# Anttwo/SuGaR

Measured on AMD Instinct MI355X. Metric: train_step_images_per_sec, higher is better.
Workload: dtype f32; 1 GPU; metric: 1000000 Gaussians @ 1920x1080, SH degree 3, 3DGS train step (raster fwd -> 0.8 L1 + 0.2 DSSIM -> bwd -> Adam, 59 floats/Gaussian), 8 orbit cameras cycled; parallelism=view-sharded dp1, single process, no collective

## Files before the change

### include/sugar_raster.h

```cpp
#ifndef SUGAR_RASTER_H_INCLUDED
#define SUGAR_RASTER_H_INCLUDED

#include <stddef.h>
#include <stdint.h>

#ifdef __cplusplus
extern "C" {
#endif

#define SGR_ABI_VERSION 4

#define SGR_E_INVALID (-1)
#define SGR_E_HIP (-2)
#define SGR_E_ALLOC (-3)

typedef char* (*sgr_alloc_fn)(void* user, size_t bytes);

int sgr_abi_version(void);
const char* sgr_last_error(void);

int64_t sgr_forward(sgr_alloc_fn geom_alloc, void* geom_user,
                    sgr_alloc_fn binning_alloc, void* binning_user,
                    sgr_alloc_fn img_alloc, void* img_user,
                    int P, int D, int M,
// ... 89 lines not shown
    float* campos_row;
    int flags;
} sgr_backward_opts;
#define SGR_BWD_EXACT_ALPHA 2
#define SGR_BWD_TILE_ORDER_READY 1
#define SGR_BWD_DENSE 8
#define SGR_BWD_ACC_CLEAN 4
#define SGR_BWD_ROWS_BY_REACH 16
#define SGR_BWD_ROWS_UNKNOWN 32
int sgr_backward_ex(int phase, int P, int D, int M, int64_t R,
                    const float* background, int width, int height,
                    const float* means3D, const float* shs, const float* colors_precomp,
                    const float* scales, float scale_modifier, const float* rotations,
                    const float* cov3D_precomp, const float* viewmatrix, const float* projmatrix,
                    const float* cam_pos, float tan_fovx, float tan_fovy, const int* radii,
                    char* geom_buffer, char* binning_buffer, char* img_buffer,
                    const float* dL_dpix,
                    float* dL_dmean2D, float* dL_dconic, float* dL_dopacity, float* dL_dcolor,
                    float* dL_dmean3D, float* dL_dcov3D, float* dL_dsh, float* dL_dscale, float* dL_drot,
                    int debug, void* stream, const sgr_backward_opts* opts);

int sgr_sh_grad_from_views(int P, int n_views, int D, int M, const float* means3D, const float* campos_all,
                           const float* dcolor_all, int64_t view_stride, float* dL_dsh, void* stream);

int sgr_sh_adam_from_views(int P, int n_views, int D, int M, const float* means3D, const float* campos_all,
                           const float* dcolor_all, int64_t view_stride, float* sh_params, float* exp_avg, float* exp_avg_sq,
                           float lr_dc,
                           float lr_rest, float beta1, float beta2, float eps, int step, float grad_scale, void* stream);

int sgr_sh_adam_from_views_ex(int P, int n_views, int D, int M, const float* means3D, const float* campos_all,
                              const float* dcolor_all, int64_t view_stride, float* sh_params, float* exp_avg, float* exp_avg_sq,
                              float lr_dc, float lr_rest, float beta1, float beta2, float eps, int step, float grad_scale,
                              float* dmean_extra, void* stream);

int sgr_sh_adam_zero_grad(int P, int M, float* sh_params, float* exp_avg, float* exp_avg_sq, const uint8_t* reach, float lr_dc,
                          float lr_rest, float beta1, float beta2, float eps, int step, float grad_scale,
                          const uint32_t* guard_header, uint32_t guard_capacity, void* stream);
int sgr_sh_adam_zero_grad_persistent(int P, int M, float* sh_params, float* exp_avg, float* exp_avg_sq, const uint8_t* reach, float lr_dc,
                                     float lr_rest, float beta1, float beta2, float eps, int step, float grad_scale,
                                     const uint32_t* guard_header, uint32_t guard_capacity, int n_adam, void* stream);
int sgr_sh_adam_from_views_masked(int P, int n_views, int D, int M, const float* means3D, const float* campos_all,
                                  const float* dcolor_all, int64_t view_stride, float* sh_params, float* exp_avg, float* exp_avg_sq,
                                  float lr_dc, float lr_rest, float beta1, float beta2, float eps, int step, float grad_scale,
                                  uint8_t* reach, const uint32_t* guard_header, uint32_t guard_capacity, void* stream);
void sgr_set_adam_overlap(int on);
int sgr_get_adam_overlap(void);
size_t sgr_geom_reach_offset_bytes(int P);
void sgr_set_rows_by_reach(int on);
int sgr_get_rows_by_reach(void);
size_t sgr_geom_rowdirty_offset_bytes(int P);

int sgr_mark_visible(int P, const float* means3D, const float* viewmatrix, const float* projmatrix,
                     uint8_t* present, void* stream);

size_t sgr_geom_bytes(int P);
size_t sgr_img_bytes(int width, int height);
size_t sgr_binning_bytes(int64_t R, int width, int height);

size_t sgr_geom_rec_offset(int P);
size_t sgr_geom_acc_offset_bytes(int P);
size_t sgr_img_final_T_offset(int width, int height);
size_t sgr_img_n_contrib_offset(int width, int height);
size_t sgr_img_tile_start_offset(int width, int height);
size_t sgr_img_tile_maxc_offset(int width, int height);
size_t sgr_img_tile_walked_offset(int width, int height);
size_t sgr_img_header_offset(int width, int height);
size_t sgr_binning_point_list_offset(int64_t R);

#define SGR_N_STAGES 15
void sgr_profile_enable(int stage_mask);
int sgr_profile_read(double* ms_sum, int64_t* count, int n_stages);


int sgr_dist2(int P, const float* points, float* meanDists, void* stream);
int sgr_knn(int N, const float* query, int M, const float* ref, int K, float* dists, int64_t* idx, void* stream);
size_t sgr_knn_grid_scratch_bytes(int M);
int sgr_knn_grid(int N, const float* query, int M, const float* ref, int K, float* dists, int64_t* idx, char* scratch,
                 void* stream);
int sgr_dist2_grid(int P, const float* points, float* meanDists, char* scratch, void* stream);

size_t sgr_l1_ssim_scratch_bytes(int channels, int width, int height);
int sgr_l1_ssim_forward(int channels, int width, int height, const float* img, const float* gt, float lambda,
                        char* scratch, float* loss_out, void* stream);
int sgr_l1_ssim_backward(int channels, int width, int height, const float* img, const float* gt, float lambda,
                         const char* scratch, const float* grad_loss, float* grad_img, void* stream);
int sgr_l1_ssim_backward_ex(int channels, int width, int height, const float* img, const float* gt, float lambda,
                            const char* scratch, const float* grad_loss, float* grad_img, float* loss_out, void* stream);

int sgr_adam_step(long long n, float* params, const float* grads, float* exp_avg, float* exp_avg_sq, int n_seg,
                  const long long* seg_begin, const long long* seg_end, const float* seg_lr_a, const float* seg_lr_b,
                  const int* seg_period, const int* seg_split, float beta1, float beta2, float eps, int step,
                  float grad_scale, void* stream);
int sgr_adam_step_multi(int n_tensors, const long long* n, float* const* params, const float* const* grads, float* const* exp_avg,
                        float* const* exp_avg_sq, const float* lr, const float* beta1, const float* beta2, const float* eps,
                        const int* step, void* stream);
int sgr_adam_step_ex(long long n, float* params, const float* grads, float* exp_avg, float* exp_avg_sq, int n_seg,
                     const long long* seg_begin, const long long* seg_end, const float* seg_lr_a, const float* seg_lr_b,
                     const int* seg_period, const int* seg_split, float beta1, float beta2, float eps, int step,
                     float grad_scale, const float* extra, long long extra_n, void* stream);

typedef struct sgr_train_config {
    int P, D, M, width, height;
    float* flat; float* flat_grad; float* exp_avg; float* exp_avg_sq;
    long long off_xyz, off_opacity, off_scaling, off_rotation, off_features, n_small;
    float lr_xyz, lr_opacity, lr_scaling, lr_rotation, lr_features_dc, lr_features_rest;
    float beta1, beta2, eps, lambda_dssim;
// ... 281 lines not shown
```

### sugar_amd/_lib.py

```python
from __future__ import annotations

import ctypes as C
import os

_HERE = os.path.dirname(os.path.abspath(__file__))
LIB_PATH = os.environ.get("SGR_LIB_PATH") or os.path.join(_HERE, "libsugar_raster.so")

ALLOC_FN = C.CFUNCTYPE(C.c_void_p, C.c_void_p, C.c_size_t)

_vp, _i, _f, _i64, _sz = C.c_void_p, C.c_int, C.c_float, C.c_int64, C.c_size_t
SIGNATURES = {
    "sgr_abi_version": (_i, []),
    "sgr_last_error": (C.c_char_p, []),
    "sgr_set_deep_min": (None, [_i]),
    "sgr_get_deep_min": (_i, []),
    "sgr_set_exact_alpha": (None, [_i]),
    "sgr_get_exact_alpha": (_i, []),
    "sgr_forward": (_i64, [ALLOC_FN, _vp, ALLOC_FN, _vp, ALLOC_FN, _vp, _i, _i, _i, _vp, _i, _i, _vp, _vp, _vp, _vp,
                           _vp, _f, _vp, _vp, _vp, _vp, _vp, _f, _f, _i, _vp, _vp, _i, _vp]),
    "sgr_forward_ex": (_i64, [ALLOC_FN, _vp, ALLOC_FN, _vp, ALLOC_FN, _vp, _i, _i, _i, _vp, _i, _i, _vp, _vp, _vp, _vp,
                              _vp, _f, _vp, _vp, _vp, _vp, _vp, _f, _f, _i, _vp, _vp, _i, _vp, _vp]),
    "sgr_backward": (_i, [_i, _i, _i, _i64, _vp, _i, _i, _vp, _vp, _vp, _vp, _f, _vp, _vp, _vp, _vp, _vp, _f, _f, _vp,
                          _vp, _vp, _vp, _vp, _vp, _vp, _vp, _vp, _vp, _vp, _vp, _vp, _vp, _i, _vp]),
    "sgr_backward_phase": (_i, [_i, _i, _i, _i, _i64, _vp, _i, _i, _vp, _vp, _vp, _vp, _f, _vp, _vp, _vp, _vp, _vp, _f, _f, _vp,
                                _vp, _vp, _vp, _vp, _vp, _vp, _vp, _vp, _vp, _vp, _vp, _vp, _vp, _i, _vp]),
    "sgr_backward_ex": (_i, [_i, _i, _i, _i, _i64, _vp, _i, _i, _vp, _vp, _vp, _vp, _f, _vp, _vp, _vp, _vp, _vp, _f, _f, _vp,
                             _vp, _vp, _vp, _vp, _vp, _vp, _vp, _vp, _vp, _vp, _vp, _vp, _vp, _i, _vp, _vp]),
    "sgr_mark_visible": (_i, [_i, _vp, _vp, _vp, _vp, _vp]),
    "sgr_trainer_create": (_vp, [_vp]),
    "sgr_trainer_destroy": (None, [_vp]),
    "sgr_trainer_set_binning": (_i, [_vp, _vp, _sz, _i64]),
    "sgr_trainer_step": (_i, [_vp, _vp, _i, _vp, _vp]),
    "sgr_trainer_forward_valid": (_i, [_vp, _vp]),
    "sgr_trainer_last_error": (C.c_char_p, []),
    "sgr_trainer_acc_dirty": (_i, [_vp]),
    "sgr_rccl_unique_id": (_i, [_vp]),
    "sgr_trainer_comm_init": (_i, [_vp, _vp, _i, _i, _vp, _sz]),
    "sgr_trainer_comm_destroy": (_i, [_vp]),
    "sgr_trainer_comm_abort": (_i, [_vp]),
    "sgr_trainer_step_exchange": (_i, [_vp, _vp, _i, _vp]),
    "sgr_trainer_set_exchange_chunks": (_i, [_vp, _i]),
    "sgr_trainer_last_exchange_wait_ms": (C.c_double, [_vp]),
    "sgr_bin2_bytes": (_sz, [_i, _i, _i]),
    "sgr_sh_grad_from_views": (_i, [_i, _i, _i, _i, _vp, _vp, _vp, _i64, _vp, _vp]),
    "sgr_sh_adam_from_views": (_i, [_i, _i, _i, _i, _vp, _vp, _vp, _i64, _vp, _vp, _vp, _f, _f, _f, _f, _f, _i, _f, _vp]),
    "sgr_sh_adam_from_views_ex": (_i, [_i, _i, _i, _i, _vp, _vp, _vp, _i64, _vp, _vp, _vp, _f, _f, _f, _f, _f, _i, _f, _vp, _vp]),
    "sgr_sh_adam_zero_grad": (_i, [_i, _i, _vp, _vp, _vp, _vp, _f, _f, _f, _f, _f, _i, _f, _vp, C.c_uint32, _vp]),
    "sgr_sh_adam_zero_grad_persistent": (_i, [_i, _i, _vp, _vp, _vp, _vp, _f, _f, _f, _f, _f, _i, _f, _vp, C.c_uint32, _i, _vp]),
    "sgr_sh_adam_from_views_masked": (_i, [_i, _i, _i, _i, _vp, _vp, _vp, _i64, _vp, _vp, _vp, _f, _f, _f, _f, _f, _i, _f, _vp, _vp,
                                           C.c_uint32, _vp]),
    "sgr_set_adam_overlap": (None, [_i]),
    "sgr_get_adam_overlap": (_i, []),
    "sgr_geom_reach_offset_bytes": (_sz, [_i]),
    "sgr_set_rows_by_reach": (None, [_i]),
    "sgr_trainer_invalidate_rows": (None, [_vp]),
    "sgr_get_rows_by_reach": (_i, []),
    "sgr_geom_rowdirty_offset_bytes": (_sz, [_i]),
    "sgr_geom_bytes": (_sz, [_i]),
    "sgr_img_bytes": (_sz, [_i, _i]),
    "sgr_binning_bytes": (_sz, [_i64, _i, _i]),
    "sgr_geom_rec_offset": (_sz, [_i]),
    "sgr_geom_acc_offset_bytes": (_sz, [_i]),
    "sgr_img_final_T_offset": (_sz, [_i, _i]),
    "sgr_img_n_contrib_offset": (_sz, [_i, _i]),
    "sgr_img_tile_start_offset": (_sz, [_i, _i]),
    "sgr_img_tile_maxc_offset": (_sz, [_i, _i]),
    "sgr_img_tile_walked_offset": (_sz, [_i, _i]),
    "sgr_img_header_offset": (_sz, [_i, _i]),
    "sgr_binning_point_list_offset": (_sz, [_i64]),
    "sgr_profile_enable": (None, [_i]),
    "sgr_profile_read": (_i, [_vp, _vp, _i]),
    "sgr_l1_ssim_scratch_bytes": (_sz, [_i, _i, _i]),
    "sgr_l1_ssim_forward": (_i, [_i, _i, _i, _vp, _vp, _f, _vp, _vp, _vp]),
    "sgr_l1_ssim_backward": (_i, [_i, _i, _i, _vp, _vp, _f, _vp, _vp, _vp, _vp]),
    "sgr_l1_ssim_backward_ex": (_i, [_i, _i, _i, _vp, _vp, _f, _vp, _vp, _vp, _vp, _vp]),
    "sgr_adam_step": (_i, [C.c_longlong, _vp, _vp, _vp, _vp, _i, _vp, _vp, _vp, _vp, _vp, _vp, _f, _f, _f, _i, _f, _vp]),
    "sgr_adam_step_multi": (_i, [_i, _vp, _vp, _vp, _vp, _vp, _vp, _vp, _vp, _vp, _vp, _vp]),
    "sgr_adam_step_ex": (_i, [C.c_longlong, _vp, _vp, _vp, _vp, _i, _vp, _vp, _vp, _vp, _vp, _vp, _f, _f, _f, _i, _f, _vp, C.c_longlong, _vp]),
    "sgr_density_field_forward": (_i, [_i, _i, _vp, _vp, _vp, _vp, _vp, _f, _vp, _vp, _vp, _vp]),
    "sgr_density_field_backward": (_i, [_i, _i, _vp, _vp, _vp, _vp, _vp, _f, _vp, _vp, _vp, _vp, _vp, _vp, _vp, _vp]),
    "sgr_density_field_backward_scratch_bytes": (_sz, [_i, _i, _i]),
# ... 170 lines not shown
```

### sugar_amd/csrc/binning.hip

```cpp
#include "sgr_device.h"
#include <cstdlib>

namespace {

#define WAVE_FENCE()                                          \
    do {                                                      \
        __builtin_amdgcn_fence(__ATOMIC_ACQ_REL, "wavefront"); \
        __builtin_amdgcn_wave_barrier();                      \
    } while (0)

#define LDS_ORDER()                          \
    do {                                     \
        asm volatile("" ::: "memory");       \
        __builtin_amdgcn_wave_barrier();     \
    } while (0)

#ifndef RS_ITEMS
#define RS_ITEMS 4096
#endif

struct RsParams { uint32_t kmin, kmax1 , skip3 , pad; };

__device__ __forceinline__ uint32_t rs_digit(uint32_t key, uint32_t kmin, uint32_t kmax1, int shift)
{
    return (((key == 0xFFFFFFFFu ? kmax1 : key) - kmin) >> shift) & 255u;
}

#define RS_FLAG_A 0x40000000u
#define RS_FLAG_P 0x80000000u
#define RS_VALUE 0x3FFFFFFFu
#define RS_COUNTER_WORDS (4 * 256 + 4)
#ifndef RS_LOOKBACK
#define RS_LOOKBACK 8
#endif

__device__ __forceinline__ uint32_t rs_peek(const uint32_t* p) { return __hip_atomic_load(p, __ATOMIC_RELAXED, __HIP_MEMORY_SCOPE_AGENT); }
__device__ __forceinline__ void rs_post(uint32_t* p, uint32_t v) { __hip_atomic_store(p, v, __ATOMIC_RELAXED, __HIP_MEMORY_SCOPE_AGENT); }

__global__ void __launch_bounds__(256) k_rs_prepare(int n, const uint32_t* __restrict__ keys, int n_chunks, uint32_t* __restrict__ status,
                                                    const uint2* __restrict__ minmax, int n_minmax, RsParams* __restrict__ params,
                                                    uint32_t* __restrict__ counters, int allow_skip)
{
    __shared__ uint32_t s_h[4][256];
    __shared__ uint32_t s_mm[2][4];
    uint32_t lo = 0xFFFFFFFFu, hi = 0u;
    for (int base = 0; base < n_minmax; base += 256 * 16) {
        uint2 v[16];
#pragma unroll
        for (int j = 0; j < 16; j++) v[j] = minmax[min(base + j * 256 + (int)threadIdx.x, n_minmax - 1)];
#pragma unroll
        for (int j = 0; j < 16; j++) { lo = min(lo, v[j].x); hi = max(hi, v[j].y); }
    }
    for (int o = 32; o > 0; o >>= 1) {
        lo = min(lo, (uint32_t)__shfl_xor((int)lo, o));
        hi = max(hi, (uint32_t)__shfl_xor((int)hi, o));
    }
    if ((threadIdx.x & 63) == 0) { s_mm[0][threadIdx.x >> 6] = lo; s_mm[1][threadIdx.x >> 6] = hi; }
    s_h[0][threadIdx.x] = 0; s_h[1][threadIdx.x] = 0; s_h[2][threadIdx.x] = 0; s_h[3][threadIdx.x] = 0;
    __syncthreads();
    lo = min(min(s_mm[0][0], s_mm[0][1]), min(s_mm[0][2], s_mm[0][3]));
    hi = max(max(s_mm[1][0], s_mm[1][1]), max(s_mm[1][2], s_mm[1][3]));
    if (lo > hi) { lo = 0u; hi = 0u; }
    const uint32_t kmin = lo, kmax1 = hi + 1u;
    const bool skip3 = allow_skip && ((kmax1 - kmin) >> 24) == 0u;
    if (blockIdx.x == 0 && threadIdx.x == 0) {
        RsParams pr; pr.kmin = kmin; pr.kmax1 = kmax1; pr.skip3 = skip3 ? 1u : 0u; pr.pad = 0u;
        *params = pr;
    }
#pragma unroll
    for (int p = 0; p < 4; p++) status[((size_t)p * n_chunks + blockIdx.x) * 256 + threadIdx.x] = 0u;
    const int base = blockIdx.x * RS_ITEMS;
    uint32_t kk[RS_ITEMS / 256];
#pragma unroll
    for (int i = 0; i < RS_ITEMS / 256; i++) kk[i] = keys[min(base + i * 256 + (int)threadIdx.x, n - 1)];
#pragma unroll
    for (int i = 0; i < RS_ITEMS / 256; i++) {
        const int k = base + i * 256 + threadIdx.x;
        if (k < n) {
            const uint32_t key = kk[i];
            const uint32_t nk = (key == 0xFFFFFFFFu ? kmax1 : key) - kmin;
            atomicAdd(&s_h[0][nk & 255u], 1u);
            atomicAdd(&s_h[1][(nk >> 8) & 255u], 1u);
            atomicAdd(&s_h[2][(nk >> 16) & 255u], 1u);
            if (!skip3) atomicAdd(&s_h[3][nk >> 24], 1u);
        }
    }
    __syncthreads();
#pragma unroll
    for (int p = 0; p < 4; p++) {
        const uint32_t c = s_h[p][threadIdx.x];
        if (c) atomicAdd(&counters[p * 256 + threadIdx.x], c);
    }
}

#ifndef RS_WAVES
#define RS_WAVES 16
#endif
#define RS_THREADS (64 * RS_WAVES)
__global__ void __launch_bounds__(RS_THREADS) k_rs_pass(int n, const uint32_t* __restrict__ keys_in, const uint32_t* __restrict__ vals_in,
                                                 uint32_t* __restrict__ keys_out, uint32_t* __restrict__ vals_out, int shift,
                                                 int n_chunks, uint32_t* __restrict__ status, uint32_t* __restrict__ counters,
                                                 const uint2* __restrict__ aux_by_val, uint2* __restrict__ aux_out,
                                                 const RsParams* __restrict__ params, int pass,
                                                 uint32_t* __restrict__ keys_out_skip, uint32_t* __restrict__ vals_out_skip)
{
    const RsParams pr = *params;
    if (pass == 3 && pr.skip3) return;
    if (pass == 2) {
        if (pr.skip3) { keys_out = keys_out_skip; vals_out = vals_out_skip; }
        else aux_out = nullptr;
    }
    const uint32_t kmin = pr.kmin, kmax1 = pr.kmax1;
    __shared__ uint32_t s_cnt[RS_WAVES][256];
    __shared__ uint32_t s_loc[256];
    __shared__ uint32_t s_base[256];
    __shared__ uint32_t s_scan[8];
    __shared__ uint32_t s_k[RS_ITEMS], s_v[RS_ITEMS];
    __shared__ int s_chunk;
    const int tid = threadIdx.x, wave = tid >> 6, lane = tid & 63;
    if (tid == 0) s_chunk = (int)atomicAdd(&counters[4 * 256 + pass], 1u);
    for (int i = tid; i < RS_WAVES * 256; i += RS_THREADS) (&s_cnt[0][0])[i] = 0u;
    __syncthreads();
    const int chunk = s_chunk;
    const int base = chunk * RS_ITEMS;
    const unsigned long long below = (lane == 0) ? 0ull : (~0ull >> (64 - lane));
    constexpr int G = RS_ITEMS / RS_THREADS;
    uint32_t rk[G], rv[G];
#pragma unroll
    for (int i = 0; i < G; i++) {
        const int k = base + wave * (RS_ITEMS / RS_WAVES) + i * 64 + lane;
        rk[i] = (k < n) ? keys_in[k] : 0xFFFFFFFFu;
        rv[i] = (k < n) ? (vals_in ? vals_in[k] : (uint32_t)k) : 0u;
    }
    uint32_t lrank[G];
#pragma unroll
    for (int i = 0; i < G; i++) {
        const int k = base + wave * (RS_ITEMS / RS_WAVES) + i * 64 + lane;
        const bool live = k < n;
        const uint32_t digit = rs_digit(rk[i], kmin, kmax1, shift);
        unsigned long long same = __ballot(live);
#pragma unroll
        for (int b = 0; b < 8; b++) {
            const bool bit = (digit >> b) & 1u;
            const unsigned long long bal = __ballot(bit);
            same &= bit ? bal : ~bal;
        }
        const uint32_t prev = s_cnt[wave][digit];
        lrank[i] = prev + (uint32_t)__popcll(same & below);
        WAVE_FENCE();
        if (live && (same & below) == 0ull) s_cnt[wave][digit] = prev + (uint32_t)__popcll(same);
        WAVE_FENCE();
    }
    __syncthreads();
    const bool owner = tid < 256;
    uint32_t mine = 0, tot = 0, i_mine = 0, i_tot = 0;
    uint32_t* st = status + (size_t)pass * n_chunks * 256 + (owner ? tid : 0);
    if (owner) {
#pragma unroll
        for (int w = 0; w < RS_WAVES; w++) mine += s_cnt[w][tid];
        rs_post(st + (size_t)chunk * 256, mine | (chunk == 0 ? RS_FLAG_P : RS_FLAG_A));
        tot = counters[pass * 256 + tid];
        i_mine = sgr_wave_incl_scan(mine); i_tot = sgr_wave_incl_scan(tot);
        if (lane == 63) { s_scan[wave] = i_mine; s_scan[4 + wave] = i_tot; }
    }
    __syncthreads();
    if (owner) {
        uint32_t loc = i_mine - mine, gbase = i_tot - tot;
#pragma unroll
        for (int w = 0; w < 3; w++)
            if (w < wave) { loc += s_scan[w]; gbase += s_scan[4 + w]; }
        uint32_t prefix = 0;
        int k = chunk - 1;
        bool done = k < 0;
        while (!done) {
            uint32_t v[RS_LOOKBACK];
#pragma unroll
            for (int j = 0; j < RS_LOOKBACK; j++) v[j] = (k - j >= 0) ? rs_peek(st + (size_t)(k - j) * 256) : RS_FLAG_P;
            bool stalled = false;
            int adv = 0;
#pragma unroll
            for (int j = 0; j < RS_LOOKBACK; j++) {
                if (!done && !stalled) {
                    if (v[j] == 0u) stalled = true;
                    else { prefix += v[j] & RS_VALUE; adv++; done = (v[j] & RS_FLAG_P) != 0u; }
                }
            }
            k -= adv;
        }
        if (chunk != 0) rs_post(st + (size_t)chunk * 256, (prefix + mine) | RS_FLAG_P);
        s_loc[tid] = loc;
        s_base[tid] = gbase + prefix;
        uint32_t run = loc;
#pragma unroll
        for (int w = 0; w < RS_WAVES; w++) { const uint32_t c = s_cnt[w][tid]; s_cnt[w][tid] = run; run += c; }
    }
    __syncthreads();
#pragma unroll
    for (int i = 0; i < G; i++) {
        const int k = base + wave * (RS_ITEMS / RS_WAVES) + i * 64 + lane;
        if (k < n) {
            const uint32_t digit = rs_digit(rk[i], kmin, kmax1, shift);
            const uint32_t pos = s_cnt[wave][digit] + lrank[i];
            s_k[pos] = rk[i]; s_v[pos] = rv[i];
        }
    }
    __syncthreads();
    const int live_n = min(RS_ITEMS, n - base);
#pragma unroll
    for (int i = 0; i < G; i++) {
        const int j = i * RS_THREADS + tid;
        if (j < live_n) {
            const uint32_t key = s_k[j], val = s_v[j];
            const uint32_t digit = rs_digit(key, kmin, kmax1, shift);
            const uint32_t dst = s_base[digit] + ((uint32_t)j - s_loc[digit]);
            keys_out[dst] = key;
            vals_out[dst] = val;
            if (aux_out) aux_out[dst] = aux_by_val[val];
        }
    }
}

__global__ void __launch_bounds__(256) k_bin_count(int P, int gx, int gy, int per_slice, const uint2* __restrict__ rects,
                                                   uint32_t* __restrict__ blk_hist)
{
    extern __shared__ __attribute__((aligned(16))) uint32_t s_cnt[];
    const int T = gx * gy;
    const int tid = threadIdx.x;
    for (int t = tid; t < T; t += 256) s_cnt[t] = 0u;
    __syncthreads();
    const int begin = blockIdx.x * per_slice;
    const int end = min(P, begin + per_slice);
    for (int s = begin + tid; s < end; s += 256) {
        const uint2 r = rects[s];
        const int w = (int)(r.y & 0xFFFFu), h = (int)(r.y >> 16);
        const int minx = (int)(r.x & 0xFFFFu), miny = (int)(r.x >> 16);
        for (int y = 0; y < h; y++) {
            uint32_t* rowp = s_cnt + (miny + y) * gx + minx;
            for (int x = 0; x < w; x++) atomicAdd(&rowp[x], 1u);
        }
    }
    __syncthreads();
    uint32_t* row = blk_hist + (size_t)blockIdx.x * T;
// ... 125 lines not shown
        __syncthreads();
        if (wave == 0) {
            const uint32_t a0 = s_seg[2 * lane], a1 = s_seg[2 * lane + 1];
            const uint32_t p = sgr_wave_incl_scan(a0 + a1);
            s_seg[2 * lane] = p - a0 - a1;
            s_seg[2 * lane + 1] = p - a1;
            if (lane == 63) s_total = p;
        }
        __syncthreads();
#pragma unroll
        for (int j = 0; j < 8; j++) {
            const int i = base + j * 1024 + tid;
            if (i < T) {
                tile_start[i] = carry + s_seg[j * 16 + wave] + incl[j] - c[j]; tile_maxc[i] = 0u; tile_walked[i] = 0u;
                if (repair_flag) repair_flag[i] = 0u;
            }
        }
        carry += s_total;
        __syncthreads();
    }
    for (int o = 32; o > 0; o >>= 1) mx = max(mx, (uint32_t)__shfl_xor((int)mx, o));
    for (int o = 32; o > 0; o >>= 1) exact += __shfl_xor(exact, o);
    __shared__ unsigned long long s_exact[16];
    if (lane == 0) { s_max[wave] = mx; s_exact[wave] = exact; }
    __syncthreads();
    if (tid == 0) {
        uint32_t m = 0;
        unsigned long long total = 0ull;
        for (int w = 0; w < 16; w++) { m = max(m, s_max[w]); total += s_exact[w]; }
        if (total >= 0xFFFFFFFFull) carry = 0xFFFFFFFFu;
        tile_start[T] = carry;
        header[SGR_HDR_R] = carry;
        header[SGR_HDR_R_HI] = (uint32_t)(total >> 32);
        header[SGR_HDR_MAXCOUNT] = m;
        header[SGR_HDR_HINT_MISS] = 0;
        if (clear_b2_words) { header[4] = 0; header[5] = 0; header[6] = 0; }
        header[7] = 0;
        header[SGR_HDR_DEEP] = 0;
        const uint32_t w4 = clear_b2_words ? 0u : header[4], w5 = clear_b2_words ? 0u : header[5], w6 = clear_b2_words ? 0u : header[6];
        for (int k = 0; k < 2; k++) {
            uint32_t* h = k ? host_b : host_a;
            if (!h) continue;
            h[0] = carry; h[1] = m; h[2] = (uint32_t)(total >> 32); h[3] = 0; h[4] = w4; h[5] = w5; h[6] = w6; h[7] = 0;
        }
    }
}

}

static size_t sort_state_bytes(int P)
{
    const size_t n = (size_t)(P > 0 ? P : 1);
    const size_t chunks = (n + RS_ITEMS - 1) / RS_ITEMS;
    return sgr_align(chunks * 256 * 4 * 4) + sgr_align(RS_COUNTER_WORDS * 4);
}

static size_t sort_base_bytes(int P)
{
    const size_t n = (size_t)(P > 0 ? P : 1);
    return sgr_align(n * 4) * 4 + sort_state_bytes(P) + 2 * sgr_align(n * 8);
}

size_t sgr_sort_minmax_offset(int P)
{
    const size_t n = (size_t)(P > 0 ? P : 1);
    return sort_base_bytes(P) + 2 * sgr_align(n * 4);
}

size_t sgr_sort_scratch_bytes(int P)
{
    const size_t n = (size_t)(P > 0 ? P : 1);
    return sgr_sort_minmax_offset(P) + sgr_align((n + 255) / 256 * 8) + 256;
}

size_t sgr_sort_rect_by_id_offset(int P)
{
    const size_t n = (size_t)(P > 0 ? P : 1);
    return sgr_sort_rects_offset(P) + sgr_align(n * 8);
}

size_t sgr_sort_rects_offset(int P)
{
    const size_t n = (size_t)(P > 0 ? P : 1);
    return sgr_align(n * 4) * 4 + sort_state_bytes(P);
}

size_t sgr_sort_counters_offset(int P)
{
    const size_t n = (size_t)(P > 0 ? P : 1);
    const size_t chunks = (n + RS_ITEMS - 1) / RS_ITEMS;
    return sgr_align(n * 4) * 4 + sgr_align(chunks * 256 * 4 * 4);
}
int sgr_sort_counter_words() { return RS_COUNTER_WORDS; }

void sgr_launch_gaussian_sort(int P, char* sort_scratch, const uint32_t** order_out, const uint2* rect_by_id, uint2* rects_sorted,
                              hipStream_t s, int part)
{
    const size_t n = (size_t)P;
    const size_t arr = sgr_align(n * 4);
    uint32_t* keys_a = reinterpret_cast<uint32_t*>(sort_scratch);
    uint32_t* keys_b = reinterpret_cast<uint32_t*>(sort_scratch + arr);
    uint32_t* vals_a = reinterpret_cast<uint32_t*>(sort_scratch + 2 * arr);
    uint32_t* vals_b = reinterpret_cast<uint32_t*>(sort_scratch + 3 * arr);
    uint32_t* status = reinterpret_cast<uint32_t*>(sort_scratch + 4 * arr);
    const int chunks = (P + RS_ITEMS - 1) / RS_ITEMS;
    uint32_t* counters = reinterpret_cast<uint32_t*>(sort_scratch + sgr_sort_counters_offset(P));
    uint32_t* keys_c = reinterpret_cast<uint32_t*>(sort_scratch + sort_base_bytes(P));
    uint32_t* vals_c = reinterpret_cast<uint32_t*>(sort_scratch + sort_base_bytes(P) + arr);
    const uint2* minmax = reinterpret_cast<const uint2*>(sort_scratch + sgr_sort_minmax_offset(P));
    const int n_minmax = (P + 255) / 256;
    RsParams* params = reinterpret_cast<RsParams*>(sort_scratch + sgr_sort_minmax_offset(P) + sgr_align((size_t)n_minmax * 8));
    const uint32_t* kin[4] = {keys_a, keys_b, keys_c, keys_b};
    const uint32_t* vin[4] = {nullptr, vals_b, vals_c, vals_b};
    uint32_t* kout[4] = {keys_b, keys_c, keys_b, keys_a};
    uint32_t* vout[4] = {vals_b, vals_c, vals_b, vals_a};
    static const int allow_skip = getenv("SGR_SORT_FOUR_PASSES") ? 0 : 1;
    if (part != 2)
        hipLaunchKernelGGL(k_rs_prepare, dim3(chunks), dim3(256), 0, s, P, keys_a, chunks, status, minmax, n_minmax, params, counters, allow_skip);
    for (int pass = (part == 2 ? 2 : 0); pass < (part == 1 ? 2 : 4); pass++)
        hipLaunchKernelGGL(k_rs_pass, dim3(chunks), dim3(RS_THREADS), 0, s, P, kin[pass], vin[pass], kout[pass], vout[pass], 8 * pass, chunks,
                           status, counters, rect_by_id, pass >= 2 ? rects_sorted : (uint2*)nullptr, params, pass, keys_a, vals_a);
    *order_out = vals_a;
}

static void set_lds_limit(const void* fn, size_t bytes, size_t& configured)
{
    if (bytes > configured) {
        (void)hipFuncSetAttribute(fn, hipFuncAttributeMaxDynamicSharedMemorySize, (int)bytes);
        configured = bytes;
    }
}

void sgr_launch_bin_count(int P, int gx, int gy, int n_slices, int per_slice, const uint32_t* order, const uint2* rects,
                          uint32_t* blk_hist, hipStream_t s)
{
    (void)order;
    static size_t configured = 0;
    const size_t bytes = (size_t)gx * gy * 4;
    set_lds_limit(reinterpret_cast<const void*>(&k_bin_count), bytes, configured);
    hipLaunchKernelGGL(k_bin_count, dim3(n_slices), dim3(256), bytes, s, P, gx, gy, per_slice, rects, blk_hist);
}

void sgr_launch_bin_scatter(int P, int gx, int gy, int n_slices, int per_slice, const uint32_t* order, const uint2* rects,
                            const uint32_t* tile_start, uint32_t* blk_hist, uint32_t* point_list, hipStream_t s)
{
    static size_t configured = 0;
    const size_t bytes = (size_t)gx * gy * 4;
    set_lds_limit(reinterpret_cast<const void*>(&k_bin_scatter), bytes, configured);
    hipLaunchKernelGGL(k_bin_scatter, dim3(n_slices), dim3(64), bytes, s, P, gx, gy, per_slice, order, rects, tile_start, blk_hist,
                       point_list);
}

void sgr_launch_hist_scan(int T, int n_blocks, uint32_t* blk_hist, uint32_t* tile_count, hipStream_t s)
{
    hipLaunchKernelGGL(k_hist_scan, dim3((T + 63) / 64), dim3(64), 0, s, T, n_blocks, blk_hist, tile_count);
}

void sgr_launch_tile_scan(int T, const uint32_t* tile_count, uint32_t* tile_start, uint32_t* header, uint32_t* tile_maxc,
                          uint32_t* tile_walked, int clear_b2_words, uint32_t* host_a, uint32_t* host_b, hipStream_t s, uint32_t* repair_flag)
{
    hipLaunchKernelGGL(k_tile_scan, dim3(1), dim3(1024), 0, s, T, tile_count, tile_start, header, tile_maxc, tile_walked,
                       clear_b2_words, host_a, host_b, repair_flag);
}
```

### sugar_amd/csrc/capi.hip

```cpp
#include "../../include/sugar_raster.h"
#include "sgr_common.h"
#include "tile_order.h"

#include <cstdlib>
#include <mutex>
#include <string>
#include <vector>

namespace {

thread_local std::string g_err;

int fail(int code, const std::string& msg)
{
    g_err = msg;
    return code;
}

#define HIP_TRY(expr)                                                                                   \
    do {                                                                                                \
        hipError_t e_ = (expr);                                                                         \
        if (e_ != hipSuccess)                                                                           \
            return fail(SGR_E_HIP, std::string(#expr) + ": " + hipGetErrorString(e_));                  \
    } while (0)
// ... 91 lines not shown
}

extern "C" {

int sgr_abi_version(void) { return SGR_ABI_VERSION; }
size_t sgr_geom_rowdirty_offset_bytes(int P) { return sgr_geom_rowdirty_offset(P); }
size_t sgr_geom_reach_offset_bytes(int P) { return sgr_geom_reach_offset(P); }
void sgr_set_deep_min(int entries) { g_deep_min = entries > 0 ? entries : 0; }
int sgr_get_deep_min(void) { return (int)sgr_deep_min(); }
void sgr_set_exact_alpha(int on) { g_exact_alpha = on ? 1 : 0; }
int sgr_get_exact_alpha(void) { return sgr_exact_alpha(); }

const char* sgr_last_error(void) { return g_err.c_str(); }

size_t sgr_geom_bytes(int P) { return sgr_geom_total(P); }
size_t sgr_img_bytes(int width, int height) { return sgr_img_layout(width, height).total; }
size_t sgr_binning_bytes(int64_t R, int width, int height) { return sgr_bin_layout(R, sgr_img_layout(width, height).T).total; }
size_t sgr_geom_rec_offset(int) { return 0; }
size_t sgr_geom_acc_offset_bytes(int P) { return sgr_geom_acc_offset(P); }
size_t sgr_img_final_T_offset(int w, int h) { return sgr_img_layout(w, h).final_T; }
size_t sgr_img_n_contrib_offset(int w, int h) { return sgr_img_layout(w, h).n_contrib; }
size_t sgr_img_tile_start_offset(int w, int h) { return sgr_img_layout(w, h).tile_start; }
size_t sgr_img_tile_maxc_offset(int w, int h) { return sgr_img_layout(w, h).tile_maxc; }
size_t sgr_img_tile_walked_offset(int w, int h) { return sgr_img_layout(w, h).tile_walked; }
size_t sgr_img_header_offset(int w, int h) { return sgr_img_layout(w, h).header; }
size_t sgr_binning_point_list_offset(int64_t R) { return sgr_bin_layout(R, 0).point_list; }

void sgr_profile_enable(int stage_mask) { g_prof.mask = (unsigned)stage_mask; }

int sgr_profile_read(double* ms_sum, int64_t* count, int n_stages)
{
    std::lock_guard<std::mutex> lk(g_prof_mu);
    for (int i = 0; i < n_stages; i++) { ms_sum[i] = 0.0; count[i] = 0; }
    for (auto& r : g_prof.recs) {
        float ms = 0.f;
        hipError_t e = hipEventSynchronize(r.b);
        if (e == hipSuccess) e = hipEventElapsedTime(&ms, r.a, r.b);
        if (e == hipSuccess && r.stage < n_stages) { ms_sum[r.stage] += ms; count[r.stage]++; }
        g_prof.pool.push_back(r.a); g_prof.pool.push_back(r.b);
    }
    g_prof.recs.clear();
    return 0;
}

int sgr_mark_visible(int P, const float* means3D, const float* viewmatrix, const float* projmatrix, uint8_t* present,
                     void* stream)
{
    (void)projmatrix;
    hipStream_t s = (hipStream_t)stream;
    if (P < 0) return fail(SGR_E_INVALID, "P < 0");
    sgr_launch_mark_visible(P, means3D, viewmatrix, present, s);
    hipError_t e = hipGetLastError();
    if (e != hipSuccess) return fail(SGR_E_HIP, std::string("mark_visible: ") + hipGetErrorString(e));
    return 0;
}

int64_t sgr_forward_ex(sgr_alloc_fn geom_alloc, void* geom_user, sgr_alloc_fn binning_alloc, void* binning_user,
                       sgr_alloc_fn img_alloc, void* img_user, int P, int D, int M, const float* background, int width,
                       int height, const float* means3D, const float* shs, const float* colors_precomp,
                       const float* opacities, const float* scales, float scale_modifier, const float* rotations,
                       const float* cov3D_precomp, const float* viewmatrix, const float* projmatrix, const float* cam_pos,
                       float tan_fovx, float tan_fovy, int prefiltered, float* out_color, int* radii, int debug,
                       void* stream, const sgr_forward_opts* opts)
{
    (void)prefiltered;
    hipStream_t s = (hipStream_t)stream;
    static const sgr_forward_opts no_opts = {0, 0, nullptr, nullptr, nullptr, nullptr, 0.f, 0u, nullptr};
    if (!opts) opts = &no_opts;
    int64_t binning_capacity = opts->binning_capacity;
    const int flags = opts->flags;
    const int binning_mode = (flags & SGR_FLAG_SINGLE_LEVEL_BINNING) ? 1 : 0;
    const int exact = (sgr_exact_alpha() || (flags & SGR_FLAG_EXACT_ALPHA)) ? 1 : 0;
    if (opts->tile_need && binning_mode == 1) return fail(SGR_E_INVALID, "the walk hint needs the two-level binning");
    if (P <= 0 || width <= 0 || height <= 0) return fail(SGR_E_INVALID, "P, width and height must be positive");
    if (!means3D || !opacities || !viewmatrix || !projmatrix || !background || !out_color)
        return fail(SGR_E_INVALID, "null required pointer");
    if (!shs && !colors_precomp) return fail(SGR_E_INVALID, "need SHs or precomputed colours");
    if (shs && !colors_precomp && (M <= 0 || M > 16 || (D + 1) * (D + 1) > M || D < 0 || D > 3))
        return fail(SGR_E_INVALID, "SH degree / coefficient count out of range (D <= 3, (D+1)^2 <= M <= 16)");
    if (shs && !colors_precomp && !cam_pos) return fail(SGR_E_INVALID, "cam_pos required with SHs");
    if (!cov3D_precomp && (!scales || !rotations)) return fail(SGR_E_INVALID, "need scales+rotations or cov3D_precomp");

    const ImgLayout IL = sgr_img_layout(width, height);
    const bool legacy_ok = IL.n_blocks > 0;
    if (IL.gx > 65535 || IL.gy > 65535) return fail(SGR_E_INVALID, "image too large: more than 65535 tiles per axis");
    if (!legacy_ok && binning_mode == 1)
        return fail(SGR_E_INVALID, "image too large for the single-level binning (one LDS counter per tile, about 38 000 tiles)");
    const Bin2Layout B2 = sgr_bin2_layout(P, IL.gx, IL.gy);
    char* geom = geom_alloc(geom_user, sgr_geom_bytes(P));
    char* img = img_alloc(img_user, IL.total + B2.total);
    if (!geom || !img) return fail(SGR_E_ALLOC, "geometry/image scratch allocation failed");

    GeomRec* rec = reinterpret_cast<GeomRec*>(geom);
    float* final_T = reinterpret_cast<float*>(img + IL.final_T);
    uint32_t* n_contrib = reinterpret_cast<uint32_t*>(img + IL.n_contrib);
    uint32_t* tile_start = reinterpret_cast<uint32_t*>(img + IL.tile_start);
    uint32_t* tile_cursor = reinterpret_cast<uint32_t*>(img + IL.tile_cursor);
    uint32_t* tile_maxc = reinterpret_cast<uint32_t*>(img + IL.tile_maxc);
    uint32_t* tile_walked = reinterpret_cast<uint32_t*>(img + IL.tile_walked);
    uint32_t* blk_nb = reinterpret_cast<uint32_t*>(img + IL.blk_nb);
    uint32_t* header = reinterpret_cast<uint32_t*>(img + IL.header);
    uint32_t* repair_flag = reinterpret_cast<uint32_t*>(img + IL.repair_flag);
    uint32_t* repair_list = reinterpret_cast<uint32_t*>(img + IL.repair_list);

    uint8_t* reach = (flags & SGR_FLAG_REACH) ? reinterpret_cast<uint8_t*>(geom + sgr_geom_reach_offset(P)) : nullptr;
    uint32_t* blk_hist = reinterpret_cast<uint32_t*>(img + IL.blk_hist);
// ... 395 lines not shown
```

### sugar_amd/csrc/sgr_common.h

```cpp
#pragma once
#include <cmath>
#include <cstdio>
#include <cstdlib>
#include <hip/hip_runtime.h>
#include <stdint.h>
#include <stddef.h>
#include "../../include/sugar_raster.h"

#define SGR_TILE_X 16
#define SGR_TILE_Y 16
#define SGR_TILE_PIX 256
#define SGR_NUM_CUS 256
#define SGR_LEGACY_LDS_BYTES (150 * 1024)
#define SGR_BIN_SLICES 1024

struct GeomRec {
    float x, y, cx, cy;
    float cz, opacity, depth;
    int radius;
    float r, g, b;
    uint32_t clamped;
};
static_assert(sizeof(GeomRec) == 48, "GeomRec must be 48 bytes");

// ... 140 lines not shown
        const double d = strtod(buf, nullptr);
        if ((float)d == x) { out = d; break; }
    }
    memo_x[1] = memo_x[0]; memo_d[1] = memo_d[0]; memo_x[0] = x; memo_d[0] = out;
    return out;
}
static inline float sgr_one_minus(float beta) { return (float)(1.0 - sgr_intended_double(beta)); }
static inline void sgr_bias_corrections(float beta1, float beta2, int step, float* bc1, float* bc2_sqrt)
{
    *bc1 = (float)(1.0 - pow(sgr_intended_double(beta1), (double)step));
    *bc2_sqrt = (float)sqrt(1.0 - pow(sgr_intended_double(beta2), (double)step));
}

struct SgrShAdamHyper {
    float lr_dc, lr_rest, beta1, beta2, eps, grad_scale;
    const uint32_t* guard; uint32_t guard_cap;
    float omb1, omb2, bc1, bc2_sqrt;
};
static inline SgrShAdamHyper sgr_sh_adam_hyper(float lr_dc, float lr_rest, float beta1, float beta2, float eps, int step, float grad_scale,
                                               const uint32_t* guard = nullptr, uint32_t guard_cap = 0)
{
    SgrShAdamHyper h = {lr_dc, lr_rest, beta1, beta2, eps, grad_scale, guard, guard_cap, sgr_one_minus(beta1), sgr_one_minus(beta2), 0.f, 0.f};
    sgr_bias_corrections(beta1, beta2, step, &h.bc1, &h.bc2_sqrt);
    return h;
}

void sgr_launch_sh_adam_from_views(int P, int V, int D, int M, size_t vstride, const float* means3D, const float* campos,
                                   const float* dcolor, float* sh, float* exp_avg, float* exp_avg_sq, const SgrShAdamHyper& h,
                                   float* dmean_extra, uint8_t* reach, hipStream_t s);
struct SgrShAdamJob {
    int P;
    int n_adam;
    float* sh; float* exp_avg; float* exp_avg_sq;
    const uint8_t* reach;
    float lr_dc, lr_rest, b1, b2, omb1, omb2, eps, bc1, bc2_sqrt, grad_scale;
    float zero;
    const uint32_t* guard; uint32_t guard_cap;
};
static inline SgrShAdamJob sgr_sh_adam_job(const SgrShAdamHyper& h, int P, int n_adam, float* sh, float* exp_avg, float* exp_avg_sq,
                                           const uint8_t* reach)
{
    return {P, n_adam, sh, exp_avg, exp_avg_sq, reach, h.lr_dc, h.lr_rest, h.beta1, h.beta2, h.omb1, h.omb2, h.eps, h.bc1, h.bc2_sqrt,
            h.grad_scale, 0.f, h.guard, h.guard_cap};
}
void sgr_launch_sh_adam_zero(const SgrShAdamJob& job, hipStream_t s);
void sgr_launch_sh_adam_zero_persistent(const SgrShAdamJob& job, hipStream_t s);
int sgr_adam_launch(long long n, float* params, const float* grads, float* exp_avg, float* exp_avg_sq, int n_seg,
                    const long long* seg_begin, const long long* seg_end, const float* seg_lr_a, const float* seg_lr_b,
                    const int* seg_period, const int* seg_split, float beta1, float beta2, float eps, int step, float grad_scale,
                    const float* extra, long long extra_n, const uint32_t* guard, uint32_t guard_cap, hipStream_t s);

void sgr_launch_gaussian_sort(int P, char* sort_scratch, const uint32_t** order_out, const uint2* rect_by_id, uint2* rects_sorted,
                              hipStream_t s, int part = 0);
size_t sgr_sort_rect_by_id_offset(int P);
size_t sgr_sort_minmax_offset(int P);
size_t sgr_sort_counters_offset(int P);
int sgr_sort_counter_words();
void sgr_launch_bin_count(int P, int gx, int gy, int n_slices, int per_slice, const uint32_t* order, const uint2* rects,
                          uint32_t* blk_hist, hipStream_t s);
void sgr_launch_bin_scatter(int P, int gx, int gy, int n_slices, int per_slice, const uint32_t* order, const uint2* rects,
                            const uint32_t* tile_start, uint32_t* blk_hist, uint32_t* point_list, hipStream_t s);
void sgr_launch_hist_scan(int T, int n_blocks, uint32_t* blk_hist, uint32_t* tile_count, hipStream_t s);
void sgr_launch_tile_scan(int T, const uint32_t* tile_count, uint32_t* tile_start, uint32_t* header, uint32_t* tile_maxc,
                          uint32_t* tile_walked, int clear_b2_words, uint32_t* host_a, uint32_t* host_b, hipStream_t s,
                          uint32_t* repair_flag = nullptr);

void sgr_launch_blend_fwd(int W, int H, int gx, int gy, const uint32_t* tile_start, const uint32_t* point_list,
                          const GeomRec* rec, const float* bg, float* final_T, uint32_t* n_contrib, uint32_t* tile_maxc,
                          uint32_t* tile_walked, float* out_color, unsigned long long* blk_mask, uint32_t* blk_nb,
                          uint32_t* header, uint32_t list_cap, const uint32_t* tile_need, const uint32_t* launch_order, hipStream_t s,
                          uint32_t* repair_flag = nullptr, uint32_t* repair_list = nullptr, int exact = 0, uint32_t deep_min = 0u,
                          uint8_t* reach = nullptr);
void sgr_launch_deep_list(int gx, int gy, const uint32_t* tile_start, const uint32_t* tile_need, uint32_t deep_min, uint32_t* header,
                          uint32_t list_cap, uint32_t* deep_list, hipStream_t s);
void sgr_launch_blend_fwd_deep(int W, int H, int gx, int gy, const uint32_t* tile_start, const uint32_t* point_list, const GeomRec* rec,
                               const float* bg, float* final_T, uint32_t* n_contrib, uint32_t* tile_maxc, uint32_t* tile_walked,
                               float* out_color, unsigned long long* blk_mask, uint32_t* blk_nb, uint32_t* header, uint32_t list_cap,
                               const uint32_t* tile_need, uint32_t* deep_list, uint32_t deep_min, hipStream_t s, uint32_t* repair_flag,
                               uint32_t* repair_list, int exact);
int sgr_exact_alpha();
uint32_t sgr_deep_min();
#define SGR_REPAIR_TILES 1024
void sgr_launch_blend_fwd_repair(int W, int H, int gx, int gy, const uint32_t* tile_start, const uint32_t* point_list,
                                 const GeomRec* rec, const float* bg, float* final_T, uint32_t* n_contrib, uint32_t* tile_maxc,
                                 uint32_t* tile_walked, float* out_color, unsigned long long* blk_mask, uint32_t* blk_nb,
                                 uint32_t* header, uint32_t list_cap, const uint32_t* repair_list, hipStream_t s, int exact = 0,
                                 uint8_t* reach = nullptr);
void sgr_launch_blend_fwd_post(int gx, int gy, const uint32_t* tile_maxc, const uint32_t* tile_walked, uint32_t* header, uint32_t list_cap,
                               uint32_t* tile_need_out, float hint_margin, uint32_t* header_host_dev, uint32_t* order_scratch,
                               uint32_t* order_out, hipStream_t s);
void sgr_launch_blend_bwd(int W, int H, int gx, int gy, const uint32_t* tile_start, const uint32_t* point_list,
                          const char* binning, const uint32_t* blk_nb, const GeomRec* rec, const float* bg,
                          const float* final_T, const uint32_t* n_contrib, const float* dL_dpix, float* acc,
                          const uint32_t* tile_maxc, const uint32_t* header, uint32_t list_cap, uint32_t* tile_order, int order_ready,
                          hipStream_t s, int exact = 0, const SgrShAdamJob* job = nullptr);
int sgr_backward_job(int phase, int P, int D, int M, int64_t R, const float* background, int width, int height, const float* means3D,
                     const float* shs, const float* scales, const float* rotations, const float* viewmatrix, const float* projmatrix,
                     const float* cam_pos, float tan_fovx, float tan_fovy, char* geom_buffer, char* binning_buffer, char* img_buffer,
                     const float* dL_dpix, float* dL_dmean2D, float* dL_dopacity, float* dL_dcolor, float* dL_dmean3D, float* dL_dscale,
                     float* dL_drot, void* stream, const sgr_backward_opts* opts, const SgrShAdamJob* job);
struct SgrTileOrderJob;
extern "C" int sgr_l1_ssim_forward_job(int channels, int width, int height, const float* img, const float* gt, float lambda, char* scratch,
                                       float* loss_out, const SgrTileOrderJob* job, void* stream);
extern "C" int sgr_forward_post_job(int width, int height, char* img_buffer, int64_t R, const sgr_forward_opts* opts, SgrTileOrderJob* job);
#define SGR_FORWARD_INVALID(hdr, cap) ((hdr)[SGR_HDR_R] > (cap) || (hdr)[SGR_HDR_HINT_MISS] != 0u || (hdr)[4 + SGR_B2_HDR_OVERFLOW] != 0u)
```

Baseline: 1114 images/s.

## Use two-level grouped decoupled lookback in radix sort; expose depth sort API

```diff
diff --git a/include/sugar_raster.h b/include/sugar_raster.h
--- a/include/sugar_raster.h
+++ b/include/sugar_raster.h
@@ -165,6 +165,10 @@
 
 int sgr_mark_visible(int P, const float* means3D, const float* viewmatrix, const float* projmatrix,
                      uint8_t* present, void* stream);
+
+size_t sgr_depth_sort_scratch_bytes(int P);
+int sgr_depth_sort_pairs(int P, const uint32_t* keys, const uint32_t* rect_by_id, char* sort_scratch, uint32_t* order_out,
+                         uint32_t* keys_out, uint32_t* rects_out, void* stream);
 
 size_t sgr_geom_bytes(int P);
 size_t sgr_img_bytes(int width, int height);
diff --git a/sugar_amd/_lib.py b/sugar_amd/_lib.py
--- a/sugar_amd/_lib.py
+++ b/sugar_amd/_lib.py
@@ -27,6 +27,8 @@
     "sgr_backward_ex": (_i, [_i, _i, _i, _i, _i64, _vp, _i, _i, _vp, _vp, _vp, _vp, _f, _vp, _vp, _vp, _vp, _vp, _f, _f, _vp,
                              _vp, _vp, _vp, _vp, _vp, _vp, _vp, _vp, _vp, _vp, _vp, _vp, _vp, _i, _vp, _vp]),
     "sgr_mark_visible": (_i, [_i, _vp, _vp, _vp, _vp, _vp]),
+    "sgr_depth_sort_scratch_bytes": (_sz, [_i]),
+    "sgr_depth_sort_pairs": (_i, [_i, _vp, _vp, _vp, _vp, _vp, _vp, _vp]),
     "sgr_trainer_create": (_vp, [_vp]),
     "sgr_trainer_destroy": (None, [_vp]),
     "sgr_trainer_set_binning": (_i, [_vp, _vp, _sz, _i64]),
diff --git a/sugar_amd/csrc/binning.hip b/sugar_amd/csrc/binning.hip
--- a/sugar_amd/csrc/binning.hip
+++ b/sugar_amd/csrc/binning.hip
@@ -30,9 +30,9 @@
 #define RS_FLAG_P 0x80000000u
 #define RS_VALUE 0x3FFFFFFFu
 #define RS_COUNTER_WORDS (4 * 256 + 4)
-#ifndef RS_LOOKBACK
+#define RS_GROUP 8
 #define RS_LOOKBACK 8
-#endif
+#define RS_GROUPS(chunks) (((chunks) + RS_GROUP - 1) / RS_GROUP)
 
 __device__ __forceinline__ uint32_t rs_peek(const uint32_t* p) { return __hip_atomic_load(p, __ATOMIC_RELAXED, __HIP_MEMORY_SCOPE_AGENT); }
 __device__ __forceinline__ void rs_post(uint32_t* p, uint32_t v) { __hip_atomic_store(p, v, __ATOMIC_RELAXED, __HIP_MEMORY_SCOPE_AGENT); }
@@ -69,6 +69,11 @@
     }
 #pragma unroll
     for (int p = 0; p < 4; p++) status[((size_t)p * n_chunks + blockIdx.x) * 256 + threadIdx.x] = 0u;
+    const int n_groups = RS_GROUPS(n_chunks);
+    if ((int)blockIdx.x < n_groups) {
+#pragma unroll
+        for (int p = 0; p < 4; p++) status[((size_t)4 * n_chunks + (size_t)p * n_groups + blockIdx.x) * 256 + threadIdx.x] = 0u;
+    }
     const int base = blockIdx.x * RS_ITEMS;
     uint32_t kk[RS_ITEMS / 256];
 #pragma unroll
@@ -91,6 +96,27 @@
         const uint32_t c = s_h[p][threadIdx.x];
         if (c) atomicAdd(&counters[p * 256 + threadIdx.x], c);
     }
+}
+
+__global__ void __launch_bounds__(256) k_rs_seed(int n, const uint32_t* __restrict__ keys, uint32_t* __restrict__ keys_a,
+                                                 uint2* __restrict__ minmax, uint32_t* __restrict__ counters)
+{
+    __shared__ uint32_t s_mm[2][4];
+    if (blockIdx.x == 0)
+        for (int i = threadIdx.x; i < RS_COUNTER_WORDS; i += 256) counters[i] = 0u;
+    const int k = blockIdx.x * 256 + threadIdx.x;
+    const uint32_t key = (k < n) ? keys[k] : 0xFFFFFFFFu;
+    if (k < n) keys_a[k] = key;
+    uint32_t lo = key, hi = key == 0xFFFFFFFFu ? 0u : key;
+    for (int o = 32; o > 0; o >>= 1) {
+        lo = min(lo, (uint32_t)__shfl_xor((int)lo, o));
+        hi = max(hi, (uint32_t)__shfl_xor((int)hi, o));
+    }
+    if ((threadIdx.x & 63) == 0) { s_mm[0][threadIdx.x >> 6] = lo; s_mm[1][threadIdx.x >> 6] = hi; }
+    __syncthreads();
+    if (threadIdx.x == 0)
+        minmax[blockIdx.x] = make_uint2(min(min(s_mm[0][0], s_mm[0][1]), min(s_mm[0][2], s_mm[0][3])),
+                                        max(max(s_mm[1][0], s_mm[1][1]), max(s_mm[1][2], s_mm[1][3])));
 }
 
 #ifndef RS_WAVES
@@ -158,7 +184,7 @@
     if (owner) {
 #pragma unroll
         for (int w = 0; w < RS_WAVES; w++) mine += s_cnt[w][tid];
-        rs_post(st + (size_t)chunk * 256, mine | (chunk == 0 ? RS_FLAG_P : RS_FLAG_A));
+        rs_post(st + (size_t)chunk * 256, mine | RS_FLAG_A);
         tot = counters[pass * 256 + tid];
         i_mine = sgr_wave_incl_scan(mine); i_tot = sgr_wave_incl_scan(tot);
         if (lane == 63) { s_scan[wave] = i_mine; s_scan[4 + wave] = i_tot; }
@@ -169,25 +195,46 @@
 #pragma unroll
         for (int w = 0; w < 3; w++)
             if (w < wave) { loc += s_scan[w]; gbase += s_scan[4 + w]; }
-        uint32_t prefix = 0;
-        int k = chunk - 1;
+        const int grp = chunk / RS_GROUP, pos = chunk % RS_GROUP;
+        const uint32_t* cw = st + (size_t)(chunk - pos) * 256;
+        uint32_t* gw = status + ((size_t)4 * n_chunks + (size_t)pass * RS_GROUPS(n_chunks)) * 256 + tid;
+        uint32_t v[RS_GROUP - 1], u[RS_LOOKBACK];
+        int k = grp - 1;
+#pragma unroll
+        for (int j = 0; j < RS_GROUP - 1; j++) v[j] = (j < pos) ? rs_peek(cw + (size_t)j * 256) : RS_FLAG_A;
+#pragma unroll
+        for (int j = 0; j < RS_LOOKBACK; j++) u[j] = (k - j >= 0) ? rs_peek(gw + (size_t)(k - j) * 256) : RS_FLAG_P;
+        for (bool missing = true; missing;) {
+            missing = false;
+#pragma unroll
+            for (int j = 0; j < RS_GROUP - 1; j++)
+                if (v[j] == 0u) { v[j] = rs_peek(cw + (size_t)j * 256); missing |= v[j] == 0u; }
+        }
+        uint32_t inner = 0;
+#pragma unroll
+        for (int j = 0; j < RS_GROUP - 1; j++) inner += v[j] & RS_VALUE;
+        const bool closes = pos == RS_GROUP - 1;
+        if (closes) rs_post(gw + (size_t)grp * 256, (inner + mine) | (grp == 0 ? RS_FLAG_P : RS_FLAG_A));
+        uint32_t outer = 0;
         bool done = k < 0;
         while (!done) {
-            uint32_t v[RS_LOOKBACK];
-#pragma unroll
-            for (int j = 0; j < RS_LOOKBACK; j++) v[j] = (k - j >= 0) ? rs_peek(st + (size_t)(k - j) * 256) : RS_FLAG_P;
             bool stalled = false;
             int adv = 0;
 #pragma unroll
             for (int j = 0; j < RS_LOOKBACK; j++) {
                 if (!done && !stalled) {
-                    if (v[j] == 0u) stalled = true;
-                    else { prefix += v[j] & RS_VALUE; adv++; done = (v[j] & RS_FLAG_P) != 0u; }
+                    if (u[j] == 0u) stalled = true;
+                    else { outer += u[j] & RS_VALUE; adv++; done = (u[j] & RS_FLAG_P) != 0u; }
                 }
             }
             k -= adv;
-        }
-        if (chunk != 0) rs_post(st + (size_t)chunk * 256, (prefix + mine) | RS_FLAG_P);
+            if (!done) {
+#pragma unroll
+                for (int j = 0; j < RS_LOOKBACK; j++) u[j] = (k - j >= 0) ? rs_peek(gw + (size_t)(k - j) * 256) : RS_FLAG_P;
+            }
+        }
+        if (closes && grp != 0) rs_post(gw + (size_t)grp * 256, (outer + inner + mine) | RS_FLAG_P);
+        const uint32_t prefix = outer + inner;
         s_loc[tid] = loc;
         s_base[tid] = gbase + prefix;
         uint32_t run = loc;
@@ -419,7 +466,7 @@
 {
     const size_t n = (size_t)(P > 0 ? P : 1);
     const size_t chunks = (n + RS_ITEMS - 1) / RS_ITEMS;
-    return sgr_align(chunks * 256 * 4 * 4) + sgr_align(RS_COUNTER_WORDS * 4);
+    return sgr_align((chunks + RS_GROUPS(chunks)) * 256 * 4 * 4) + sgr_align(RS_COUNTER_WORDS * 4);
 }
 
 static size_t sort_base_bytes(int P)
@@ -456,7 +503,7 @@
 {
     const size_t n = (size_t)(P > 0 ? P : 1);
     const size_t chunks = (n + RS_ITEMS - 1) / RS_ITEMS;
-    return sgr_align(n * 4) * 4 + sgr_align(chunks * 256 * 4 * 4);
+    return sgr_align(n * 4) * 4 + sgr_align((chunks + RS_GROUPS(chunks)) * 256 * 4 * 4);
 }
 int sgr_sort_counter_words() { return RS_COUNTER_WORDS; }
 
@@ -490,6 +537,18 @@
     *order_out = vals_a;
 }
 
+void sgr_launch_sort_pairs(int P, const uint32_t* keys, const uint2* rect_by_id, char* sort_scratch, uint32_t* order_out,
+                           uint32_t* keys_out, uint2* rects_out, hipStream_t s)
+{
+    hipLaunchKernelGGL(k_rs_seed, dim3((P + 255) / 256), dim3(256), 0, s, P, keys, reinterpret_cast<uint32_t*>(sort_scratch),
+                       reinterpret_cast<uint2*>(sort_scratch + sgr_sort_minmax_offset(P)),
+                       reinterpret_cast<uint32_t*>(sort_scratch + sgr_sort_counters_offset(P)));
+    const uint32_t* order = nullptr;
+    sgr_launch_gaussian_sort(P, sort_scratch, &order, rect_by_id, rect_by_id ? rects_out : nullptr, s);
+    (void)hipMemcpyAsync(order_out, order, (size_t)P * 4, hipMemcpyDeviceToDevice, s);
+    (void)hipMemcpyAsync(keys_out, sort_scratch, (size_t)P * 4, hipMemcpyDeviceToDevice, s);
+}
+
 static void set_lds_limit(const void* fn, size_t bytes, size_t& configured)
 {
     if (bytes > configured) {
diff --git a/sugar_amd/csrc/capi.hip b/sugar_amd/csrc/capi.hip
--- a/sugar_amd/csrc/capi.hip
+++ b/sugar_amd/csrc/capi.hip
@@ -167,6 +167,21 @@
     sgr_launch_mark_visible(P, means3D, viewmatrix, present, s);
     hipError_t e = hipGetLastError();
     if (e != hipSuccess) return fail(SGR_E_HIP, std::string("mark_visible: ") + hipGetErrorString(e));
+    return 0;
+}
+
+size_t sgr_depth_sort_scratch_bytes(int P) { return sgr_sort_scratch_bytes(P); }
+
+int sgr_depth_sort_pairs(int P, const uint32_t* keys, const uint32_t* rect_by_id, char* sort_scratch, uint32_t* order_out,
+                         uint32_t* keys_out, uint32_t* rects_out, void* stream)
+{
+    if (P < 1) return fail(SGR_E_INVALID, "P < 1");
+    if (!keys || !sort_scratch || !order_out || !keys_out || (rect_by_id && !rects_out))
+        return fail(SGR_E_INVALID, "sgr_depth_sort_pairs: null buffer");
+    sgr_launch_sort_pairs(P, keys, reinterpret_cast<const uint2*>(rect_by_id), sort_scratch, order_out, keys_out,
+                          reinterpret_cast<uint2*>(rects_out), (hipStream_t)stream);
+    hipError_t e = hipGetLastError();
+    if (e != hipSuccess) return fail(SGR_E_HIP, std::string("depth_sort_pairs: ") + hipGetErrorString(e));
     return 0;
 }
 
diff --git a/sugar_amd/csrc/sgr_common.h b/sugar_amd/csrc/sgr_common.h
--- a/sugar_amd/csrc/sgr_common.h
+++ b/sugar_amd/csrc/sgr_common.h
@@ -216,6 +216,8 @@
 
 void sgr_launch_gaussian_sort(int P, char* sort_scratch, const uint32_t** order_out, const uint2* rect_by_id, uint2* rects_sorted,
                               hipStream_t s, int part = 0);
+void sgr_launch_sort_pairs(int P, const uint32_t* keys, const uint2* rect_by_id, char* sort_scratch, uint32_t* order_out,
+                           uint32_t* keys_out, uint2* rects_out, hipStream_t s);
 size_t sgr_sort_rect_by_id_offset(int P);
 size_t sgr_sort_minmax_offset(int P);
 size_t sgr_sort_counters_offset(int P);
```

Result: no change. 1119 images/s, median of 6 (+0.5%).
